# pqpeqr/RL-2048-with-Reinforce-and-Actor-Critic

Hardware: NVIDIA B200
Metric: 2048 env-steps/sec (random-legal batched env stepping, 1M packed boards per GPU) (higher is better)
Workload: dtype u64

## Files before the change

### profiles/sass_pipes.py

```python
#!/usr/bin/env python
import collections, os, re, subprocess, sys

ROOT = os.path.dirname(os.path.dirname(os.path.abspath(__file__)))
DEFAULT_LIB = os.path.join(ROOT, "rl-2048-with-reinforce-and-actor-critic_b200", "libb2048.so")
DEFAULT_KERNELS = ["_ZN2b216step_fast_kernelILi3ELb1ELb1EEEvNS_8StepArgsE"]

ALU = {"LOP3", "LOP", "SHF", "SHL", "SHR", "SEL", "FSEL", "ISETP", "FSETP", "IADD3", "IADD", "VIADD", "VIADDMNMX", "LEA",
       "PRMT", "POPC", "FLO", "BREV", "IMNMX", "VIMNMX", "IABS", "BMSK", "SGXT", "PLOP3", "P2R", "R2P", "MOV", "ICMP",
       "ISCADD", "CS2R"}
FMA = {"IMAD", "FFMA", "FMUL", "FADD", "HFMA2", "HADD2", "HMUL2", "IDP", "IMUL"}
FP64 = {"DADD", "DMUL", "DFMA", "DSETP", "F2F", "F2I", "I2F", "I2FP", "F2FP"}
MEM = {"LDS", "LDG", "STG", "STS", "LD", "ST", "ATOM", "ATOMS", "RED", "REDG", "LDC", "LDL", "STL"}
PIPES = ["alu", "fma", "fp64/conv", "mem", "ctrl", "uniform", "other"]

LINE = re.compile(r"\s*/\*([0-9a-f]{4,})\*/\s+(@!?U?P[T0-9]+\s+)?([A-Z0-9_]+)((?:\.[A-Z0-9_]+)*)\s*([^;]*);")


def pipe(op):
    if op in ALU:
        return "alu"
    if op in FMA:
        return "fma"
    if op in FP64:
        return "fp64/conv"
    if op in MEM:
        return "mem"
    if op in {"BRA", "BSSY", "BSYNC", "EXIT", "NOP", "WARPSYNC", "YIELD", "BAR", "PREEXIT", "CALL", "RET", "BPT"}:
        return "ctrl"
    if op.startswith("U") or op in {"S2UR", "R2UR", "S2R", "CS2R"}:
        return "uniform"
    return "other"


def sass_of(path, kernel):
    out = subprocess.run(["cuobjdump", "-sass", "-fun", kernel, path], capture_output=True, text=True)
    if out.returncode != 0 or "Function" not in out.stdout:
        sys.exit(f"cuobjdump found no function {kernel} in {path}:\n{out.stderr}")
    ins = []
    for line in out.stdout.splitlines():
        m = LINE.match(line)
        if m:
            ins.append((int(m.group(1), 16), m.group(3), m.group(3) + m.group(4), m.group(5), bool(m.group(2))))
    return ins


def regions(ins):
    idx = {a[0]: k for k, a in enumerate(ins)}
    best = None
    for a, op, full, arg, pred in ins:
        if op == "BRA" and pred:
            m = re.search(r"0x([0-9a-f]+)", arg)
            tgt = int(m.group(1), 16) if m else None
            if tgt is not None and tgt < a and tgt in idx and (best is None or a - tgt > best[1] - best[0]):
                best = (tgt, a)
    if best is None:
        sys.exit("no loop found")
    lo, hi = idx[best[0]], idx[best[1]]
    first_st = next((k for k in range(lo, hi + 1) if ins[k][1] in ("STG", "ST")), hi + 1)
    blocks = []
    for k in range(lo, first_st):
        a, op, full, arg, pred = ins[k]
        if op == "BSSY":
            m = re.search(r"(B\d+),\s*0x([0-9a-f]+)", arg)
            end = int(m.group(2), 16)
            if end in idx and idx[end] <= first_st:
                blocks.append((k, idx[end]))
    reset = max(blocks, key=lambda b: b[1] - b[0], default=None)
    in_reset = set(range(reset[0], reset[1] + 1)) if reset else set()
    return {"main": [ins[k] for k in range(lo, first_st) if k not in in_reset],
            "reset": [ins[k] for k in sorted(in_reset)],
            "tail": [ins[k] for k in range(first_st, hi + 1)]}


def main():
    args = [a for a in sys.argv[1:] if a != "-v"]
    verbose = "-v" in sys.argv[1:]
    path = args[0] if args else DEFAULT_LIB
    kernels = args[1:] or DEFAULT_KERNELS
    for kern in kernels:
        regs = regions(sass_of(path, kern))
        print(f"{kern}")
        print(f"{'region':8s} {'instrs':>6s} " + " ".join(f"{p:>9s}" for p in PIPES))
        tot = collections.Counter()
        for name, body in regs.items():
            c = collections.Counter(pipe(x[1]) for x in body)
            tot.update(c)
            print(f"{name:8s} {len(body):6d} " + " ".join(f"{c[p]:9d}" for p in PIPES))
        print(f"{'loop':8s} {sum(tot.values()):6d} " + " ".join(f"{tot[p]:9d}" for p in PIPES))
        if verbose:
            for name, body in regs.items():
                c = collections.Counter(x[2] for x in body)
                print(f"  {name}: " + ", ".join(f"{k} {v}" for k, v in c.most_common()))


if __name__ == "__main__":
    main()
```

### rl-2048-with-reinforce-and-actor-critic_b200/csrc/b2048_env.cu

```cuda
#include <cuda_runtime.h>

#include <cstdio>
#include <cstdlib>

#include "b2048_internal.h"
#include "b2048_ptx.cuh"
#include "b2048_step_fast.cuh"

namespace b2 {

__global__ void build_lut_kernel(uint16_t* __restrict__ lut_left, uint8_t* __restrict__ lut_merge) {
    uint32_t row = blockIdx.x * blockDim.x + threadIdx.x;
    if (row >= 65536u) return;
    uint32_t out, merge;
    row_move_left(row, out, merge);
    lut_left[row] = (uint16_t)out;
    lut_merge[row] = (uint8_t)merge;
}

__global__ void build_small_tables_kernel(uint8_t* __restrict__ small) {
    static_assert(B2048_SMALL_BYTES == B2048_TABLES_BYTES - B2048_LUT_BYTES, "small table size mismatch");
    const uint32_t tid = threadIdx.x;
    if (tid < 256u) small_table_entry_agg(tid, reinterpret_cast<AggEntry*>(small + B2048_SMALL_AGG_OFF)[tid]);
    if (tid < 4u) small_table_entry_sel(tid, reinterpret_cast<SelEntry*>(small + B2048_SMALL_SEL_OFF)[tid]);
    if (tid < 64u) small[B2048_SMALL_ACT_OFF + tid] = (uint8_t)small_table_entry_act(tid >> 2, tid & 3u);
}

__global__ void __launch_bounds__(256) reset_kernel(uint64_t* __restrict__ board, uint32_t* __restrict__ score,
                                                     uint32_t* __restrict__ step, uint8_t* __restrict__ max_exp,
                                                     uint8_t* __restrict__ flags,
                                                     const uint8_t* __restrict__ spawn_replay, int64_t n, uint64_t seed,
                                                     uint64_t gid0, uint32_t t) {
    int64_t stride = (int64_t)gridDim.x * blockDim.x;
    for (int64_t i = (int64_t)blockIdx.x * blockDim.x + threadIdx.x; i < n; i += stride) {
        Board b;
        if (spawn_replay) {
            uint32_t r0 = spawn_replay[2 * i], r1 = spawn_replay[2 * i + 1];
            b = place_kth_empty(Board{0u, 0u}, r0 & 0xFu, (r0 & 0x10u) ? 2u : 1u);
            b = place_kth_empty(b, r1 & 0xFu, (r1 & 0x10u) ? 2u : 1u);
        } else {
            b = reset_board(seed, gid0 + (uint64_t)i, t);
        }
        board[i] = to_u64(b);
        if (score) score[i] = 0u;
        if (step) step[i] = 0u;
        if (max_exp) max_exp[i] = 2u;
        if (flags) flags[i] = (uint8_t)legal_mask(b);
    }
}

__global__ void __launch_bounds__(256) np_seed_kernel(const uint64_t* __restrict__ seeds, b2048_np_rng* __restrict__ rng,
                                                       int64_t n) {
    for (int64_t i = (int64_t)blockIdx.x * blockDim.x + threadIdx.x; i < n; i += (int64_t)gridDim.x * blockDim.x)
        rng[i] = np::seed(seeds[i]);
}

__global__ void __launch_bounds__(256) reset_np_kernel(uint64_t* __restrict__ board, uint32_t* __restrict__ score,
                                                        uint32_t* __restrict__ step, uint8_t* __restrict__ max_exp,
                                                        uint8_t* __restrict__ flags, b2048_np_rng* __restrict__ env_rng,
                                                        int64_t n) {
    for (int64_t i = (int64_t)blockIdx.x * blockDim.x + threadIdx.x; i < n; i += (int64_t)gridDim.x * blockDim.x) {
        b2048_np_rng r = env_rng[i];
        const Board b = np::reset_board(r);
        env_rng[i] = r;
        board[i] = to_u64(b);
        if (score) score[i] = 0u;
        if (step) step[i] = 0u;
        if (max_exp) max_exp[i] = 2u;
        if (flags) flags[i] = (uint8_t)legal_mask(b);
    }
}

struct StepArgs {
    const uint64_t* board_in;
    uint64_t* board_out;
    uint32_t* score;
    uint32_t* step;
    uint8_t* max_exp;
    const uint8_t* action;
    uint8_t* action_out;
    const uint8_t* flags_in;
    const uint8_t* spawn_replay;
    int32_t* ep_len;
    uint32_t ep_t;
    int32_t* merge_sum;
    float* reward;
    double* reward64;
    uint8_t* flags;
    float* obs;
    const uint8_t* tables;
    int64_t n;
    uint64_t seed, gid0;
    uint32_t t;
    b2048_env_cfg cfg;
    PhiloxKeys keys;
    long long* debug_clock;
};

template <bool kSmall, class Args>
__device__ __forceinline__ void stage_tables(uint8_t* smem, const Args& args, uint64_t* mbar) {
    const uint32_t bar = s_u32(mbar);
    if (threadIdx.x == 0) {
        mbar_init(bar, 1);
        mbar_init_fence();
    }
    __syncthreads();
    if (threadIdx.x == 0) {
        mbar_expect_tx(bar, kSmall ? (uint32_t)B2048_TABLES_BYTES : (uint32_t)B2048_LUT_BYTES);
        if (kSmall) bulk_load(s_u32(smem + B2048_LUT_BYTES), args.tables + B2048_LUT_BYTES, (uint32_t)B2048_SMALL_BYTES, bar);
        bulk_load_chunked<32768u>(s_u32(smem), args.tables, (uint32_t)B2048_LUT_BYTES, bar);
    }
}

__device__ __forceinline__ void store_obs16(float* __restrict__ obs, Board nb, int64_t warp_base, int64_t n, int lane,
                                            int obs_mode, float scale) {
#pragma unroll
    for (int s = 0; s < 4; ++s) {
        int src = 8 * s + (lane >> 2);
        uint32_t lo = __shfl_sync(0xFFFFFFFFu, nb.lo, src);
        uint32_t hi = __shfl_sync(0xFFFFFFFFu, nb.hi, src);
        int row = lane & 3;
        uint32_t w = (row & 2) ? hi : lo;
        uint32_t r16 = (w >> (16 * (row & 1))) & 0xFFFFu;
        float v[4];
        encode_row(r16, obs_mode, scale, v);
        int64_t bi = warp_base + src;
        if (bi < n) {
            float4 q = make_float4(v[0], v[1], v[2], v[3]);
            *reinterpret_cast<float4*>(obs + bi * 16 + row * 4) = q;
        }
    }
}

__device__ __forceinline__ void store_obs_onehot(float* __restrict__ obs, Board nb, int64_t warp_base, int64_t n,
                                                 int lane) {
    for (int j = 0; j < 32; ++j) {
        int64_t bi = warp_base + j;
        if (bi >= n) break;
        uint32_t lo = __shfl_sync(0xFFFFFFFFu, nb.lo, j);
        uint32_t hi = __shfl_sync(0xFFFFFFFFu, nb.hi, j);
        uint64_t b = (uint64_t)lo | ((uint64_t)hi << 32);
        float4* dst = reinterpret_cast<float4*>(obs + bi * 272);
#pragma unroll
        for (int q0 = 0; q0 < 96; q0 += 32) {
            int q = q0 + lane;
            if (q < 68) {
                float v[4];
#pragma unroll
                for (int u = 0; u < 4; ++u) {
                    int f = 4 * q + u;
                    int cell = f / 17, ch = f - 17 * cell;
                    int e = (int)((b >> (4 * cell)) & 0xFull);
                    v[u] = (e == ch) ? 1.0f : 0.0f;
                }
                dst[q] = make_float4(v[0], v[1], v[2], v[3]);
            }
        }
    }
}

template <bool kSmemLut, int kThreads, bool kNp>
__device__ __forceinline__ void step_loop(const StepArgs& args, b2048_np_rng* env_rng) {
    extern __shared__ __align__(128) uint8_t smem[];
    __shared__ uint64_t mbar;

    const int tid = threadIdx.x;
    __builtin_assume(tid < kThreads);
    const int lane = tid & 31;
    const uint16_t* lut_left;
    const uint8_t* lut_merge;

    if (kSmemLut) {
        stage_tables<false>(smem, args, &mbar);
        lut_left = reinterpret_cast<const uint16_t*>(smem);
        lut_merge = smem + B2048_LUT_LEFT_BYTES;
    } else {
        lut_left = reinterpret_cast<const uint16_t*>(args.tables);
        lut_merge = args.tables + B2048_LUT_LEFT_BYTES;
    }

    const b2048_env_cfg& cfg = args.cfg;
    StepOpts opt;
    opt.track_step = args.step != nullptr;
    opt.track_max = args.max_exp != nullptr;
    opt.want_sum = cfg.reward_mode == B2048_REWARD_SUM || args.score != nullptr || args.merge_sum != nullptr;

    bool lut_ready = !kSmemLut;
    const int64_t stride = (int64_t)gridDim.x * kThreads;
    for (int64_t base = (int64_t)blockIdx.x * kThreads; base < args.n; base += stride) {
        const int64_t i = base + tid;
        const bool valid = i < args.n;
        StepIO io;
        io.board = Board{0u, 0u};
        io.score = 0u;
        io.step = 0u;
        io.max_exp = 2u;
        io.action = 0u;
        io.mask_in = 0u;
        io.have_mask_in = args.flags_in != nullptr;
        io.replay = 0u;
        if (valid) {
            if (args.spawn_replay) io.replay = args.spawn_replay[i];
            io.board = make_board(args.board_in[i]);
            if (args.score) io.score = args.score[i];
            if (args.step) io.step = args.step[i];
            if (args.max_exp) io.max_exp = args.max_exp[i];
            if (cfg.action_mode == B2048_ACT_BUFFER) io.action = args.action[i];
            if (args.flags_in) io.mask_in = args.flags_in[i];
        }
        if (!lut_ready) {
            mbar_wait(s_u32(&mbar), 0);
            lut_ready = true;
        }
        bool frozen = false;
        Board board_before = io.board;
        if (args.ep_len && valid) frozen = args.ep_len[i] != 0;
        b2048_np_rng rng;
        if constexpr (kNp) {
            if (valid && !frozen) rng = env_rng[i];
        }
        step_one<decltype(lut_left), decltype(lut_merge), kNp>(io, cfg, opt, args.seed, args.gid0 + (uint64_t)i, args.t,
                                                              lut_left, lut_merge, &rng, valid && !frozen);
        if (valid && frozen) {
            uint32_t m = legal_mask(board_before);
            uint32_t f = args.flags_in ? (uint32_t)args.flags_in[i]
                                       : (m | ((m == 0u && (board_before.lo | board_before.hi) != 0u) ? B2048_F_DONE : 0u));
            args.board_out[i] = to_u64(board_before);
            if (args.action_out) args.action_out[i] = 0;
            if (args.merge_sum) args.merge_sum[i] = 0;
            if (args.reward) args.reward[i] = 0.0f;
            if (args.reward64) args.reward64[i] = 0.0;
            args.flags[i] = (uint8_t)(f & ~B2048_F_CHANGED);
            io.board = board_before;
        } else if (valid) {
            if (args.ep_len && (io.flags & (B2048_F_DONE | B2048_F_TRUNC))) args.ep_len[i] = (int32_t)args.ep_t;
            args.board_out[i] = to_u64(io.board);
            if (args.score) args.score[i] = io.score;
            if (args.step) args.step[i] = io.step;
            if (args.max_exp) args.max_exp[i] = (uint8_t)io.max_exp;
            if (args.action_out) args.action_out[i] = (uint8_t)io.action_played;
            if (args.merge_sum) args.merge_sum[i] = io.merge_sum;
            if (args.reward) args.reward[i] = (float)io.reward;
            if (args.reward64) args.reward64[i] = io.reward;
            args.flags[i] = (uint8_t)io.flags;
            if constexpr (kNp) {
                if (io.flags & B2048_F_CHANGED) env_rng[i] = rng;
            }
        }
        if (args.obs != nullptr && cfg.obs_mode != B2048_OBS_NONE) {
            const int64_t warp_base = base + (tid & ~31);
            if (cfg.obs_mode == B2048_OBS_ONEHOT) store_obs_onehot(args.obs, io.board, warp_base, args.n, lane);
            else store_obs16(args.obs, io.board, warp_base, args.n, lane, cfg.obs_mode, cfg.obs_log2_scale);
        }
    }
}

template <bool kSmemLut, int kThreads>
__global__ void __launch_bounds__(kThreads, kSmemLut ? 1 : 2) step_kernel(const __grid_constant__ StepArgs args) {
    step_loop<kSmemLut, kThreads, false>(args, nullptr);
}

template <bool kSmemLut, int kThreads>
__global__ void __launch_bounds__(kThreads, kSmemLut ? 1 : 2) step_np_kernel(const __grid_constant__ StepArgs args,
                                                                              b2048_np_rng* __restrict__ env_rng) {
    step_loop<kSmemLut, kThreads, true>(args, env_rng);
}

template <int kAct, bool kTrack, bool kPlain>
__global__ void __launch_bounds__(1024, 1) step_fast_kernel(const __grid_constant__ StepArgs args) {
    extern __shared__ __align__(128) uint8_t smem[];
    __shared__ uint64_t mbar;
    const int tid = threadIdx.x;
    const bool dbg = args.debug_clock != nullptr && tid == 0 && (blockIdx.x == 0 || blockIdx.x == 147);
    long long* dc = dbg ? args.debug_clock + (blockIdx.x == 0 ? 0 : 16) : nullptr;
    int dci = 0;
    if (dbg) { dc[dci++] = (long long)globaltimer(); dc[dci++] = clock64(); }
    pdl_launch_dependents();
    stage_tables<true>(smem, args, &mbar);
    FastTables T;
    T.left = reinterpret_cast<const uint16_t*>(smem);
    T.merge = smem + B2048_LUT_LEFT_BYTES;
    T.agg = reinterpret_cast<const AggEntry*>(smem + B2048_LUT_BYTES + B2048_SMALL_AGG_OFF);
    T.sel = reinterpret_cast<const SelEntry*>(smem + B2048_LUT_BYTES + B2048_SMALL_SEL_OFF);
    T.act = smem + B2048_LUT_BYTES + B2048_SMALL_ACT_OFF;
    pdl_wait();

    const b2048_env_cfg& cfg = args.cfg;
    if constexpr (kPlain) {
        const uint32_t n = (uint32_t)args.n, stride = gridDim.x * 1024u;
        uint32_t i = blockIdx.x * 1024u + (uint32_t)tid;
        uint2 bw_next = make_uint2(0u, 0u);
        uint32_t act_next = 0u, fin_next = 0u, score_next = 0u, step_next = 0u, max_next = 2u;
        auto request = [&](uint32_t k) {
            bw_next = *reinterpret_cast<const uint2*>(args.board_in + k);
            if (kAct == B2048_ACT_BUFFER) act_next = args.action[k];
            else if (kAct != B2048_ACT_RANDOM_ANY) fin_next = args.flags_in[k];
            if (kTrack) { score_next = args.score[k]; step_next = args.step[k]; max_next = args.max_exp[k]; }
        };
        if (i < n) request(i);
        Rand4 rnd = stream_keyed(args.keys, args.gid0 + (uint64_t)i, args.t, B2048_DOM_STEP);
        mbar_wait(s_u32(&mbar), 0);
        for (; i < n; i += stride) {
            FastIO io;
            io.lo = bw_next.x; io.hi = bw_next.y;
            io.score = score_next; io.step = step_next; io.max_exp = max_next;
            io.action = act_next; io.mask_in = fin_next;
            const uint32_t inext = i + stride;
            if (inext < n) request(inext);
            step_fast_rnd<kAct, kTrack, false>(io, cfg, rnd, args.keys, args.gid0 + (uint64_t)i, args.t, T);
            *reinterpret_cast<uint2*>(args.board_out + i) = make_uint2(io.lo, io.hi);
            if (kTrack) { args.score[i] = io.score; args.step[i] = io.step; args.max_exp[i] = (uint8_t)io.max_exp; }
            args.reward[i] = io.reward;
            args.flags[i] = (uint8_t)io.flags;
            if (inext < n) rnd = stream_keyed(args.keys, args.gid0 + (uint64_t)inext, args.t, B2048_DOM_STEP);
        }
        return;
    }
    bool ready = false;
    const int64_t stride = (int64_t)gridDim.x * 1024;
    int64_t i = (int64_t)blockIdx.x * 1024 + tid;
    uint2 bw_next = make_uint2(0u, 0u);
    uint32_t act_next = 0u, fin_next = 0u;
    if (i < args.n) {
        bw_next = *reinterpret_cast<const uint2*>(args.board_in + i);
        if (kAct == B2048_ACT_BUFFER) act_next = args.action[i];
        if (args.flags_in) fin_next = args.flags_in[i];
    }
    for (; i < args.n; i += stride) {
        FastIO io;
        const uint2 bw = bw_next;
        const uint32_t fin = fin_next;
        io.lo = bw.x; io.hi = bw.y;
        io.score = 0u; io.step = 0u; io.max_exp = 2u; io.mask_in = 0u;
        io.action = act_next;
        const int64_t inext = i + stride;
        if (inext < args.n) {
            bw_next = *reinterpret_cast<const uint2*>(args.board_in + inext);
            if (kAct == B2048_ACT_BUFFER) act_next = args.action[inext];
            if (args.flags_in) fin_next = args.flags_in[inext];
        }
        if (kTrack) { io.score = args.score[i]; io.step = args.step[i]; io.max_exp = args.max_exp[i]; }
        if (kAct == B2048_ACT_RANDOM_LEGAL || kAct == B2048_ACT_PRIORITY)
            io.mask_in = args.flags_in ? fin : legal_mask(Board{io.lo, io.hi});
        bool frozen = false;
        if (args.ep_len) frozen = args.ep_len[i] != 0;
        if (!ready) {
            mbar_wait(s_u32(&mbar), 0);
            ready = true;
            if (dbg) dc[dci++] = clock64();
        }
        if (frozen) {
            uint32_t m = legal_mask(Board{io.lo, io.hi});
            uint32_t f = args.flags_in ? fin : (m | ((m == 0u && (io.lo | io.hi) != 0u) ? B2048_F_DONE : 0u));
            *reinterpret_cast<uint2*>(args.board_out + i) = bw;
            if (args.action_out) args.action_out[i] = 0;
            if (args.merge_sum) args.merge_sum[i] = 0;
            args.reward[i] = 0.0f;
            args.flags[i] = (uint8_t)(f & ~B2048_F_CHANGED);
            continue;
        }
        step_fast<kAct, kTrack>(io, cfg, args.keys, args.seed, args.gid0 + (uint64_t)i, args.t, T);
        if (args.ep_len && (io.flags & (B2048_F_DONE | B2048_F_TRUNC))) args.ep_len[i] = (int32_t)args.ep_t;
        *reinterpret_cast<uint2*>(args.board_out + i) = make_uint2(io.lo, io.hi);
        if (kTrack) { args.score[i] = io.score; args.step[i] = io.step; args.max_exp[i] = (uint8_t)io.max_exp; }
        if (args.action_out) args.action_out[i] = (uint8_t)io.action;
        if (args.merge_sum) args.merge_sum[i] = io.merge_sum;
        args.reward[i] = io.reward;
        args.flags[i] = (uint8_t)io.flags;
        if (dbg && dci < 12) dc[dci++] = clock64();
    }
    if (dbg) { const unsigned long long gt = globaltimer(); dc[14] = clock64(); dc[15] = (long long)gt; }
}

template <int kAct, bool kTrack, bool kPlain>
static cudaError_t launch_fast_one(int grid, size_t smem, cudaStream_t s, const StepArgs& a, bool pdl) {
    cudaLaunchConfig_t lc = {};
    lc.gridDim = dim3((unsigned)grid); lc.blockDim = dim3(1024); lc.dynamicSmemBytes = smem; lc.stream = s;
    cudaLaunchAttribute at[1];
    at[0].id = cudaLaunchAttributeProgrammaticStreamSerialization;
    at[0].val.programmaticStreamSerializationAllowed = 1;
    lc.attrs = at; lc.numAttrs = pdl ? 1u : 0u;
    return cudaLaunchKernelEx(&lc, step_fast_kernel<kAct, kTrack, kPlain>, a);
}
template <int kAct>
static cudaError_t launch_fast(bool track, int grid, size_t smem, cudaStream_t s, const StepArgs& a, bool pdl) {
    const bool plain = a.ep_len == nullptr && a.action_out == nullptr && a.merge_sum == nullptr && a.debug_clock == nullptr &&
                       (kAct == B2048_ACT_BUFFER || kAct == B2048_ACT_RANDOM_ANY || a.flags_in != nullptr) &&
                       a.n < ((int64_t)1 << 31) - (int64_t)grid * 1024 &&
                       !cfg_is_shaped(a.cfg);
    if (plain) return track ? launch_fast_one<kAct, true, true>(grid, smem, s, a, pdl) : launch_fast_one<kAct, false, true>(grid, smem, s, a, pdl);
    return track ? launch_fast_one<kAct, true, false>(grid, smem, s, a, pdl) : launch_fast_one<kAct, false, false>(grid, smem, s, a, pdl);
}

struct StepNArgs {
    uint64_t* board;
    uint32_t* score;
    uint32_t* step;
    uint8_t* max_exp;
    uint8_t* flags;
    float* reward_last;
    float* reward_sum;
    int32_t* episodes;
    const uint8_t* tables;
    int64_t n;
    int32_t n_steps, flags_valid;
    uint64_t seed, gid0;
    uint32_t t;
    b2048_env_cfg cfg;
    PhiloxKeys keys;
};

template <int kAct, bool kTrack, bool kShaped>
__global__ void __launch_bounds__(1024, 1) step_fast_n_kernel(const __grid_constant__ StepNArgs args) {
    extern __shared__ __align__(128) uint8_t smem[];
    __shared__ uint64_t mbar;
    const int tid = threadIdx.x;
    stage_tables<true>(smem, args, &mbar);
    FastTables T;
    T.left = reinterpret_cast<const uint16_t*>(smem);
    T.merge = smem + B2048_LUT_LEFT_BYTES;
    T.agg = reinterpret_cast<const AggEntry*>(smem + B2048_LUT_BYTES + B2048_SMALL_AGG_OFF);
    T.sel = reinterpret_cast<const SelEntry*>(smem + B2048_LUT_BYTES + B2048_SMALL_SEL_OFF);
    T.act = smem + B2048_LUT_BYTES + B2048_SMALL_ACT_OFF;
    const b2048_env_cfg& cfg = args.cfg;
    bool ready = false;
    const int64_t stride = (int64_t)gridDim.x * 1024;
    for (int64_t i = (int64_t)blockIdx.x * 1024 + tid; i < args.n; i += stride) {
        FastIO io;
        const uint2 bw = *reinterpret_cast<const uint2*>(args.board + i);
        io.lo = bw.x; io.hi = bw.y;
        io.score = 0u; io.step = 0u; io.max_exp = 2u; io.action = 0u;
        if (kTrack) { io.score = args.score[i]; io.step = args.step[i]; io.max_exp = args.max_exp[i]; }
        io.mask_in = args.flags_valid ? (uint32_t)args.flags[i] : legal_mask(Board{io.lo, io.hi});
        io.flags = io.mask_in;
        io.reward = 0.0f;
        if (!ready) {
            mbar_wait(s_u32(&mbar), 0);
            ready = true;
        }
        float rsum = 0.0f;
        int32_t eps = 0;
        const uint64_t gid = args.gid0 + (uint64_t)i;
        for (int32_t k = 0; k < args.n_steps; ++k) {
            io.mask_in = io.flags & 0xFu;
            step_fast<kAct, kTrack, kShaped>(io, cfg, args.keys, args.seed, gid, args.t + (uint32_t)k, T);
            rsum += io.reward;
            eps += (io.flags & (B2048_F_DONE | B2048_F_TRUNC)) ? 1 : 0;
        }
        *reinterpret_cast<uint2*>(args.board + i) = make_uint2(io.lo, io.hi);
        if (kTrack) { args.score[i] = io.score; args.step[i] = io.step; args.max_exp[i] = (uint8_t)io.max_exp; }
        args.flags[i] = (uint8_t)io.flags;
        if (args.reward_last) args.reward_last[i] = io.reward;
        if (args.reward_sum) args.reward_sum[i] += rsum;
        if (args.episodes) args.episodes[i] += eps;
    }
}

__global__ void __launch_bounds__(256) move_kernel(const uint64_t* __restrict__ board_in, uint64_t* __restrict__ board_out,
                                                    const uint8_t* __restrict__ action, int32_t* __restrict__ merge_sum,
                                                    uint8_t* __restrict__ merge_info, uint8_t* __restrict__ flags,
                                                    const uint8_t* __restrict__ tables, int64_t n) {
    const uint16_t* lut_left = reinterpret_cast<const uint16_t*>(tables);
    const uint8_t* lut_merge = tables + B2048_LUT_LEFT_BYTES;
    int64_t stride = (int64_t)gridDim.x * blockDim.x;
    for (int64_t i = (int64_t)blockIdx.x * blockDim.x + threadIdx.x; i < n; i += stride) {
        Board b = make_board(board_in[i]);
        MoveResult mv = move_board(b, action[i] & 3u, lut_left, lut_merge);
        MergeStats ms = merge_stats(mv.merge, true, false);
        uint32_t mask = legal_mask(mv.board);
        bool changed = (mv.board.lo != b.lo) | (mv.board.hi != b.hi);
        bool done = (mask == 0u) & ((mv.board.lo | mv.board.hi) != 0u);
        board_out[i] = to_u64(mv.board);
        if (merge_sum) merge_sum[i] = (int32_t)ms.sum;
        if (merge_info) *reinterpret_cast<uint32_t*>(merge_info + 4 * i) = mv.merge;
        if (flags)
            flags[i] = (uint8_t)(mask | (changed ? B2048_F_CHANGED : 0u) | (done ? B2048_F_DONE : 0u) |
                                 (ms.overflow ? B2048_F_OVERFLOW : 0u));
    }
}

__global__ void __launch_bounds__(256) obs_kernel(const uint64_t* __restrict__ board, float* __restrict__ obs, int obs_mode,
                                                   float scale, int64_t n) {
    const int lane = threadIdx.x & 31;
    int64_t stride = (int64_t)gridDim.x * blockDim.x;
    for (int64_t base = (int64_t)blockIdx.x * blockDim.x; base < n; base += stride) {
        int64_t i = base + threadIdx.x;
        Board b = i < n ? make_board(board[i]) : Board{0u, 0u};
        int64_t warp_base = base + (threadIdx.x & ~31);
        if (obs_mode == B2048_OBS_ONEHOT) store_obs_onehot(obs, b, warp_base, n, lane);
        else store_obs16(obs, b, warp_base, n, lane, obs_mode, scale);
    }
}

struct SymVariant {
    uint64_t perm;
    uint32_t amap;
    uint32_t mperm;
};
__constant__ SymVariant kSym[8] = {
    {0xFEDCBA9876543210ull, 0xE4u, 0xE4u}, {0xC840D951EA62FB73ull, 0x93u, 0x39u},
    {0x0123456789ABCDEFull, 0x4Eu, 0x4Eu}, {0x37BF26AE159D048Cull, 0x39u, 0x93u},
    {0xCDEF89AB45670123ull, 0x6Cu, 0x6Cu}, {0xFB73EA62D951C840ull, 0x1Bu, 0x1Bu},
    {0x32107654BA98FEDCull, 0xC6u, 0xC6u}, {0x048C159D26AE37BFull, 0xB1u, 0xB1u},
};

__global__ void __launch_bounds__(256) symmetries_kernel(const uint64_t* __restrict__ board, const uint8_t* __restrict__ flags,
                                                          const uint8_t* __restrict__ action, uint64_t* __restrict__ board_out,
                                                          uint8_t* __restrict__ flags_out, uint8_t* __restrict__ action_out,
                                                          int64_t rows, int64_t n) {
    const int64_t total = rows * n;
    for (int64_t e = (int64_t)blockIdx.x * blockDim.x + threadIdx.x; e < total; e += (int64_t)gridDim.x * blockDim.x) {
        const int64_t r = e / n, i = e - r * n;
        const uint64_t b = board ? board[e] : 0ull;
        const uint32_t f = flags ? flags[e] : 0u, a = action ? (action[e] & 3u) : 0u;
#pragma unroll
        for (int v = 0; v < 8; ++v) {
            const SymVariant sv = kSym[v];
            const int64_t o = r * 8 * n + (int64_t)v * n + i;
            if (board_out) {
                uint64_t nb = 0;
#pragma unroll
                for (int c = 0; c < 16; ++c) nb |= ((b >> (4 * (uint32_t)((sv.perm >> (4 * c)) & 0xFull))) & 0xFull) << (4 * c);
                board_out[o] = nb;
            }
            if (flags_out) {
                uint32_t nf = f & 0xF0u;
#pragma unroll
                for (int k = 0; k < 4; ++k) nf |= ((f >> ((sv.mperm >> (2 * k)) & 3u)) & 1u) << k;
                flags_out[o] = (uint8_t)nf;
            }
            if (action_out) action_out[o] = (uint8_t)((sv.amap >> (2 * a)) & 3u);
        }
    }
}

static int grid_for(int64_t n, int threads, int num_sms, int per_sm) {
    int64_t blocks = (n + threads - 1) / threads;
    int64_t cap = (int64_t)num_sms * per_sm;
    if (blocks > cap) blocks = cap;
    if (blocks < 1) blocks = 1;
    return (int)blocks;
}

}

using namespace b2;

extern "C" int b2048_create(b2048_handle** out) {
    B2_REQUIRE(out != nullptr, "b2048_create: out is NULL");
    b2048_handle* h = new b2048_handle();
    B2_CUDA(cudaGetDevice(&h->device));
    B2_CUDA(cudaDeviceGetAttribute(&h->num_sms, cudaDevAttrMultiProcessorCount, h->device));
    B2_CUDA(cudaDeviceGetAttribute(&h->smem_optin, cudaDevAttrMaxSharedMemoryPerBlockOptin, h->device));
    B2_CUDA(cudaMalloc(&h->d_tables, B2048_TABLES_BYTES));
    build_lut_kernel<<<256, 256>>>(reinterpret_cast<uint16_t*>(h->d_tables), h->d_tables + B2048_LUT_LEFT_BYTES);
    build_small_tables_kernel<<<1, 256>>>(h->d_tables + B2048_LUT_BYTES);
    B2_CUDA(cudaGetLastError());
    B2_CUDA(cudaDeviceSynchronize());
    if (h->smem_optin >= B2048_LUT_BYTES) {
        B2_CUDA(cudaFuncSetAttribute(step_kernel<true, 1024>, cudaFuncAttributeMaxDynamicSharedMemorySize,
                                     B2048_LUT_BYTES));
        B2_CUDA(cudaFuncSetAttribute(step_np_kernel<true, 1024>, cudaFuncAttributeMaxDynamicSharedMemorySize,
                                     B2048_LUT_BYTES));
    }
    if (h->smem_optin >= B2048_TABLES_BYTES) {
#define B2_SET(A, TR)                                                                                                       \
    B2_CUDA(cudaFuncSetAttribute(step_fast_kernel<A, TR, false>, cudaFuncAttributeMaxDynamicSharedMemorySize, B2048_TABLES_BYTES)); \
    B2_CUDA(cudaFuncSetAttribute(step_fast_kernel<A, TR, true>, cudaFuncAttributeMaxDynamicSharedMemorySize, B2048_TABLES_BYTES))
        B2_SET(B2048_ACT_BUFFER, true); B2_SET(B2048_ACT_BUFFER, false);
        B2_SET(B2048_ACT_RANDOM_LEGAL, true); B2_SET(B2048_ACT_RANDOM_LEGAL, false);
        B2_SET(B2048_ACT_RANDOM_ANY, true); B2_SET(B2048_ACT_RANDOM_ANY, false);
        B2_SET(B2048_ACT_PRIORITY, true); B2_SET(B2048_ACT_PRIORITY, false);
#define B2_SET_N(A, TR)                                                                                                               \
    do {                                                                                                                              \
        B2_CUDA(cudaFuncSetAttribute(step_fast_n_kernel<A, TR, false>, cudaFuncAttributeMaxDynamicSharedMemorySize, B2048_TABLES_BYTES)); \
        B2_CUDA(cudaFuncSetAttribute(step_fast_n_kernel<A, TR, true>, cudaFuncAttributeMaxDynamicSharedMemorySize, B2048_TABLES_BYTES));  \
    } while (0)
        B2_SET_N(B2048_ACT_RANDOM_LEGAL, true); B2_SET_N(B2048_ACT_RANDOM_LEGAL, false);
        B2_SET_N(B2048_ACT_RANDOM_ANY, true); B2_SET_N(B2048_ACT_RANDOM_ANY, false);
        B2_SET_N(B2048_ACT_PRIORITY, true); B2_SET_N(B2048_ACT_PRIORITY, false);
#undef B2_SET_N
#undef B2_SET
    }
    *out = h;
    return B2048_OK;
}

extern "C" int b2048_destroy(b2048_handle* h) {
    if (!h) return B2048_OK;
    cudaFree(h->d_tables);
    if (h->tc_image) cudaFree(h->tc_image);
    if (h->hp_image) cudaFree(h->hp_image);
    if (h->gen_image) cudaFree(h->gen_image);
    if (h->dbg_clock) cudaFree(h->dbg_clock);
    if (h->dbg_progress) cudaFreeHost(h->dbg_progress);
    delete h;
    return B2048_OK;
}

extern "C" int b2048_get_row_lut(b2048_handle* h, uint16_t* lut_left_host, uint8_t* lut_merge_host) {
    B2_REQUIRE(h != nullptr, "b2048_get_row_lut: handle is NULL");
    if (lut_left_host) B2_CUDA(cudaMemcpy(lut_left_host, h->d_tables, B2048_LUT_LEFT_BYTES, cudaMemcpyDeviceToHost));
    if (lut_merge_host)
        B2_CUDA(cudaMemcpy(lut_merge_host, h->d_tables + B2048_LUT_LEFT_BYTES, B2048_LUT_MERGE_BYTES,
                           cudaMemcpyDeviceToHost));
    return B2048_OK;
}

extern "C" int b2048_reset_many(b2048_handle* h, uint64_t* board, uint32_t* score, uint32_t* step, uint8_t* max_exp,
                                uint8_t* flags, const uint8_t* spawn_replay, int64_t n, uint64_t seed, uint64_t gid0,
                                uint32_t t, void* stream) {
    B2_REQUIRE(h != nullptr, "b2048_reset_many: handle is NULL");
    B2_REQUIRE(n >= 0, "b2048_reset_many: n < 0");
    B2_REQUIRE(board != nullptr || n == 0, "b2048_reset_many: board is NULL");
    if (n == 0) return B2048_OK;
    reset_kernel<<<grid_for(n, 256, h->num_sms, 8), 256, 0, (cudaStream_t)stream>>>(board, score, step, max_exp, flags,
                                                                                   spawn_replay, n, seed, gid0, t);
    B2_CUDA(cudaGetLastError());
    return B2048_OK;
}

extern "C" int b2048_np_rng_seed(const uint64_t* seeds, b2048_np_rng* rng, int64_t n, void* stream) {
    B2_REQUIRE(n >= 0, "b2048_np_rng_seed: n < 0");
    if (n == 0) return B2048_OK;
    B2_REQUIRE(seeds && rng, "b2048_np_rng_seed: seeds / rng is NULL");
    const int64_t blocks = (n + 255) / 256;
    np_seed_kernel<<<(unsigned)(blocks < 65536 ? blocks : 65536), 256, 0, (cudaStream_t)stream>>>(seeds, rng, n);
    B2_CUDA(cudaGetLastError());
    return B2048_OK;
}

extern "C" int b2048_reset_many_np(b2048_handle* h, uint64_t* board, uint32_t* score, uint32_t* step, uint8_t* max_exp,
                                   uint8_t* flags, b2048_np_rng* env_rng, int64_t n, void* stream) {
    B2_REQUIRE(h != nullptr, "b2048_reset_many_np: handle is NULL");
    B2_REQUIRE(n >= 0, "b2048_reset_many_np: n < 0");
    if (n == 0) return B2048_OK;
    B2_REQUIRE(board && env_rng, "b2048_reset_many_np: board / env_rng is NULL");
    reset_np_kernel<<<grid_for(n, 256, h->num_sms, 8), 256, 0, (cudaStream_t)stream>>>(board, score, step, max_exp, flags,
                                                                                       env_rng, n);
    B2_CUDA(cudaGetLastError());
    return B2048_OK;
}

int b2::launch_step_np(b2048_handle* h, const uint64_t* board_in, uint64_t* board_out, uint32_t* score, uint32_t* step,
                   uint8_t* max_exp, const uint8_t* action, const uint8_t* flags_in, const b2048_env_cfg* cfg, float* reward,
                   uint8_t* flags, int32_t* ep_len, uint32_t ep_t, int64_t n, b2048_np_rng* env_rng, cudaStream_t s) {
    StepArgs a = {};
    a.board_in = board_in; a.board_out = board_out; a.score = score; a.step = step; a.max_exp = max_exp;
    a.action = action; a.flags_in = flags_in; a.ep_len = ep_len; a.ep_t = ep_t;
    a.reward = reward; a.flags = flags; a.tables = h->d_tables; a.n = n; a.cfg = *cfg;
    if (h->smem_optin >= B2048_LUT_BYTES && n >= (int64_t)32768) {
        step_np_kernel<true, 1024><<<grid_for(n, 1024, h->num_sms, 1), 1024, B2048_LUT_BYTES, s>>>(a, env_rng);
    } else {
        step_np_kernel<false, 256><<<grid_for(n, 256, h->num_sms, 8), 256, 0, s>>>(a, env_rng);
    }
    B2_CUDA(cudaGetLastError());
    return B2048_OK;
}

extern "C" int b2048_step_many(b2048_handle* h, const uint64_t* board_in, uint64_t* board_out, uint32_t* score,
                               uint32_t* step, uint8_t* max_exp, const uint8_t* action, uint8_t* action_out,
                               const uint8_t* flags_in, const uint8_t* spawn_replay, const b2048_env_cfg* cfg,
                               int32_t* merge_sum, float* reward,
                               double* reward64, uint8_t* flags, float* obs, int32_t* ep_len, uint32_t ep_t, int64_t n,
                               uint64_t seed, uint64_t gid0, uint32_t t, void* stream) {
    B2_REQUIRE(h != nullptr, "b2048_step_many: handle is NULL");
    B2_REQUIRE(cfg != nullptr, "b2048_step_many: cfg is NULL");
    B2_REQUIRE(n >= 0, "b2048_step_many: n < 0");
    if (n == 0) return B2048_OK;
    B2_REQUIRE(board_in && board_out && flags, "b2048_step_many: board_in/board_out/flags must not be NULL");
    B2_REQUIRE(cfg->reward_mode == B2048_REWARD_SUM || cfg->reward_mode == B2048_REWARD_LOG2,
               "b2048_step_many: unsupported reward mode");
    B2_REQUIRE(cfg->bonus_mode >= B2048_BONUS_OFF && cfg->bonus_mode <= B2048_BONUS_LOG2,
               "b2048_step_many: unsupported bonus mode");
    B2_REQUIRE(cfg->obs_mode >= B2048_OBS_NONE && cfg->obs_mode <= B2048_OBS_ONEHOT,
               "b2048_step_many: unsupported obs_mode");
    B2_REQUIRE(cfg->action_mode >= B2048_ACT_BUFFER && cfg->action_mode <= B2048_ACT_PRIORITY,
               "b2048_step_many: unsupported action_mode");
    B2_REQUIRE(cfg->action_mode != B2048_ACT_BUFFER || action != nullptr,
               "b2048_step_many: action buffer required for B2048_ACT_BUFFER");
    StepArgs a;
    a.board_in = board_in; a.board_out = board_out; a.score = score; a.step = step; a.max_exp = max_exp;
    a.action = action; a.action_out = action_out; a.flags_in = flags_in; a.spawn_replay = spawn_replay; a.ep_len = ep_len; a.ep_t = ep_t;
    a.merge_sum = merge_sum;
    a.reward = reward; a.reward64 = reward64; a.flags = flags; a.obs = obs; a.tables = h->d_tables;
    a.n = n; a.seed = seed; a.gid0 = gid0; a.t = t; a.cfg = *cfg; a.keys = make_keys(seed);
    cudaStream_t s = (cudaStream_t)stream;
    a.debug_clock = debug_clock_begin(h, B2048_DBG_STEP_CLOCKS, s);
    const bool use_smem = h->smem_optin >= B2048_LUT_BYTES && n >= (int64_t)32768;
    const bool all_track = score && step && max_exp, none_track = !score && !step && !max_exp;
    const bool fast = h->smem_optin >= B2048_TABLES_BYTES && n >= (int64_t)32768 && (all_track || none_track) &&
                      cfg->use_action_mask && (cfg->bonus_mode == B2048_BONUS_OFF || all_track) && reward != nullptr &&
                      reward64 == nullptr && spawn_replay == nullptr && (obs == nullptr || cfg->obs_mode == B2048_OBS_NONE) &&
                      !(h->debug & (1u << B2048_DBG_NO_FAST_STEP));
    if (fast) {
        int grid = grid_for(n, 1024, h->num_sms, 1);
        const bool pdl = !(h->debug & (1u << B2048_DBG_NO_PDL));
        cudaError_t e;
        if (cfg->action_mode == B2048_ACT_BUFFER) e = launch_fast<B2048_ACT_BUFFER>(all_track, grid, B2048_TABLES_BYTES, s, a, pdl);
        else if (cfg->action_mode == B2048_ACT_RANDOM_LEGAL) e = launch_fast<B2048_ACT_RANDOM_LEGAL>(all_track, grid, B2048_TABLES_BYTES, s, a, pdl);
        else if (cfg->action_mode == B2048_ACT_PRIORITY) e = launch_fast<B2048_ACT_PRIORITY>(all_track, grid, B2048_TABLES_BYTES, s, a, pdl);
        else e = launch_fast<B2048_ACT_RANDOM_ANY>(all_track, grid, B2048_TABLES_BYTES, s, a, pdl);
        B2_CUDA(e);
    } else if (use_smem) {
        int grid = grid_for(n, 1024, h->num_sms, 1);
        step_kernel<true, 1024><<<grid, 1024, B2048_LUT_BYTES, s>>>(a);
    } else {
        int grid = grid_for(n, 256, h->num_sms, 8);
        step_kernel<false, 256><<<grid, 256, 0, s>>>(a);
    }
    B2_CUDA(cudaGetLastError());
    if (a.debug_clock && fast) {
        long long hb[32];
        { int st = debug_clock_read(h, hb, 32, s); if (st != B2048_OK) return st; }
        for (int c = 0; c < 2; ++c) {
            long long* d = hb + 16 * c;
            fprintf(stderr, "[step clock] cta %d: start@%lld ns, staged +%lld cyc, iters:", c ? 147 : 0, d[0] - hb[0], d[2] - d[1]);
            for (int k = 3; k < 12 && d[k]; ++k) fprintf(stderr, " %lld", d[k] - d[k - 1]);
            fprintf(stderr, " | total %lld cyc, %lld ns\n", d[14] - d[1], d[15] - d[0]);
        }
    }
    return B2048_OK;
}

extern "C" int b2048_symmetries(b2048_handle* h, const uint64_t* board, const uint8_t* flags, const uint8_t* action,
                                uint64_t* board_out, uint8_t* flags_out, uint8_t* action_out, int64_t rows, int64_t n,
                                void* stream) {
    B2_REQUIRE(h != nullptr, "b2048_symmetries: handle is NULL");
    B2_REQUIRE(rows >= 0 && n >= 0, "b2048_symmetries: negative size");
    if (rows == 0 || n == 0) return B2048_OK;
    B2_REQUIRE((board == nullptr) == (board_out == nullptr) && (flags == nullptr) == (flags_out == nullptr) &&
                   (action == nullptr) == (action_out == nullptr),
               "b2048_symmetries: every input needs its output buffer and vice versa");
    symmetries_kernel<<<grid_for(rows * n, 256, h->num_sms, 8), 256, 0, (cudaStream_t)stream>>>(
        board, flags, action, board_out, flags_out, action_out, rows, n);
    B2_CUDA(cudaGetLastError());
    return B2048_OK;
}

extern "C" int b2048_step_many_n(b2048_handle* h, uint64_t* board, uint32_t* score, uint32_t* step, uint8_t* max_exp,
                                 uint8_t* flags, int32_t flags_valid, const b2048_env_cfg* cfg, float* reward_last,
                                 float* reward_sum, int32_t* episodes, int64_t n, int32_t n_steps, uint64_t seed,
                                 uint64_t gid0, uint32_t t, void* stream) {
    B2_REQUIRE(h != nullptr && cfg != nullptr, "b2048_step_many_n: handle / cfg is NULL");
    B2_REQUIRE(n >= 0 && n_steps >= 0, "b2048_step_many_n: negative size");
    if (n == 0 || n_steps == 0) return B2048_OK;
    B2_REQUIRE(board && flags, "b2048_step_many_n: board / flags must not be NULL");
    B2_REQUIRE(cfg->action_mode == B2048_ACT_RANDOM_LEGAL || cfg->action_mode == B2048_ACT_RANDOM_ANY ||
                   cfg->action_mode == B2048_ACT_PRIORITY,
               "b2048_step_many_n: needs a device-side action mode (random_legal, random_any or priority)");
    const bool all_track = score && step && max_exp, none_track = !score && !step && !max_exp;
    const bool ok = h->smem_optin >= B2048_TABLES_BYTES && (all_track || none_track) && cfg->use_action_mask &&
                    (cfg->bonus_mode == B2048_BONUS_OFF || all_track) &&
                    (cfg->reward_mode == B2048_REWARD_SUM || cfg->reward_mode == B2048_REWARD_LOG2);
    if (!ok)
        return fail(B2048_ERR_UNSUPPORTED,
                    "b2048_step_many_n: implemented for action-mask-on configurations (the new-max-tile bonus needs the "
                    "tracked counters) with score / step / max_exp all present or all absent; call "
                    "b2048_step_many n_steps times otherwise");
    StepNArgs a;
    a.board = board; a.score = score; a.step = step; a.max_exp = max_exp; a.flags = flags; a.reward_last = reward_last;
    a.reward_sum = reward_sum; a.episodes = episodes; a.tables = h->d_tables; a.n = n; a.n_steps = n_steps;
    a.flags_valid = flags_valid; a.seed = seed; a.gid0 = gid0; a.t = t; a.cfg = *cfg; a.keys = make_keys(seed);
    const int grid = grid_for(n, 1024, h->num_sms, 1);
    cudaStream_t s = (cudaStream_t)stream;
    const bool shaped = cfg_is_shaped(*cfg);
#define B2_LAUNCH_N(A)                                                                                      \
    do {                                                                                                    \
        if (all_track && shaped) step_fast_n_kernel<A, true, true><<<grid, 1024, B2048_TABLES_BYTES, s>>>(a);    \
        else if (all_track) step_fast_n_kernel<A, true, false><<<grid, 1024, B2048_TABLES_BYTES, s>>>(a);        \
        else if (shaped) step_fast_n_kernel<A, false, true><<<grid, 1024, B2048_TABLES_BYTES, s>>>(a);           \
        else step_fast_n_kernel<A, false, false><<<grid, 1024, B2048_TABLES_BYTES, s>>>(a);                      \
    } while (0)
    if (cfg->action_mode == B2048_ACT_RANDOM_LEGAL) B2_LAUNCH_N(B2048_ACT_RANDOM_LEGAL);
    else if (cfg->action_mode == B2048_ACT_PRIORITY) B2_LAUNCH_N(B2048_ACT_PRIORITY);
    else B2_LAUNCH_N(B2048_ACT_RANDOM_ANY);
#undef B2_LAUNCH_N
    B2_CUDA(cudaGetLastError());
    return B2048_OK;
}

extern "C" int b2048_move_many(b2048_handle* h, const uint64_t* board_in, uint64_t* board_out, const uint8_t* action,
                               int32_t* merge_sum, uint8_t* merge_info, uint8_t* flags, int64_t n, void* stream) {
    B2_REQUIRE(h != nullptr, "b2048_move_many: handle is NULL");
    B2_REQUIRE(n >= 0, "b2048_move_many: n < 0");
    if (n == 0) return B2048_OK;
    B2_REQUIRE(board_in && board_out && action, "b2048_move_many: board_in/board_out/action must not be NULL");
    move_kernel<<<grid_for(n, 256, h->num_sms, 8), 256, 0, (cudaStream_t)stream>>>(board_in, board_out, action, merge_sum,
                                                                                  merge_info, flags, h->d_tables, n);
    B2_CUDA(cudaGetLastError());
    return B2048_OK;
}

extern "C" int b2048_encode_obs(const uint64_t* board, float* obs, int32_t obs_mode, float obs_log2_scale, int64_t n,
                                void* stream) {
    B2_REQUIRE(n >= 0, "b2048_encode_obs: n < 0");
    B2_REQUIRE(obs_mode >= B2048_OBS_RAW && obs_mode <= B2048_OBS_ONEHOT, "b2048_encode_obs: unsupported obs_mode");
    if (n == 0) return B2048_OK;
    B2_REQUIRE(board && obs, "b2048_encode_obs: board/obs must not be NULL");
    int dev = 0, sms = 148;
    B2_CUDA(cudaGetDevice(&dev));
    B2_CUDA(cudaDeviceGetAttribute(&sms, cudaDevAttrMultiProcessorCount, dev));
    obs_kernel<<<grid_for(n, 256, sms, 8), 256, 0, (cudaStream_t)stream>>>(board, obs, obs_mode, obs_log2_scale, n);
    B2_CUDA(cudaGetLastError());
    return B2048_OK;
}
```

Baseline: 59.53 billion.

## Process two boards per thread in plain fast step path with vectorized IO

Replaces the plain specialization of the fast step kernel with a new pair kernel that runs 512 threads per block, each stepping two adjacent boards per iteration. Loads and stores use wider vector accesses (uint4 boards, uint2 score/step, 16-bit packed flags/actions) and two independent step chains per thread to raise ILP. The launch path adds alignment checks and handles an odd trailing board separately. The cost is fewer resident threads per SM and higher register pressure, and it adds slope-timing and SASS-counting scripts.

```diff
diff --git a/profiles/run_step_slope.py b/profiles/run_step_slope.py
--- /dev/null
+++ b/profiles/run_step_slope.py
@@ -0,0 +1,70 @@
+#!/usr/bin/env python
+import argparse
+import json
+import os
+import subprocess
+import sys
+
+ROOT = os.path.dirname(os.path.dirname(os.path.abspath(__file__)))
+sys.path.insert(0, ROOT)
+
+
+def gpu_info():
+    try:
+        q = subprocess.run(["nvidia-smi", "--query-gpu=name,power.limit,clocks.max.sm", "--format=csv,noheader"],
+                           capture_output=True, text=True, timeout=30)
+        return q.stdout.strip().splitlines()[0] if q.returncode == 0 and q.stdout.strip() else None
+    except (OSError, subprocess.SubprocessError):
+        return None
+
+
+def time_launch(b2048, torch, n, K, R):
+    from bench import RUNNER_ENV
+    envs = [b2048.Batched2048Env(n, b2048.Game2048EnvConfig(**RUNNER_ENV), seed=0xB200 + r, gid0=0) for r in range(R)]
+    for e in envs:
+        e.reset_many()
+        e.step_many_n(64, action_mode="random_legal", auto_reset=True)
+    for k in range(max(10, R)):
+        envs[k % R].step_many(action_mode="random_legal", auto_reset=True)
+    t0, t1 = torch.cuda.Event(enable_timing=True), torch.cuda.Event(enable_timing=True)
+    torch.cuda.synchronize()
+    torch.cuda._sleep(2_000_000)
+    t0.record()
+    for k in range(K):
+        envs[k % R].step_many(action_mode="random_legal", auto_reset=True)
+    t1.record()
+    torch.cuda.synchronize()
+    return t0.elapsed_time(t1) * 1e3 / K
+
+
+def main():
+    ap = argparse.ArgumentParser()
+    ap.add_argument("--steps", type=int, default=2000)
+    ap.add_argument("--batches", type=int, default=12)
+    ap.add_argument("--kmax", type=int, default=7)
+    ap.add_argument("--out")
+    args = ap.parse_args()
+    import numpy as np
+    import torch
+    import b2048
+    if not torch.cuda.is_available():
+        sys.exit("run_step_slope.py needs a CUDA device")
+    per_iter = torch.cuda.get_device_properties(0).multi_processor_count * 1024
+    ks = list(range(1, args.kmax + 1))
+    us = [time_launch(b2048, torch, k * per_iter, args.steps, args.batches) for k in ks]
+    b, a = np.polyfit(ks, us, 1)
+    resid = np.asarray(us) - (a + b * np.asarray(ks))
+    line = {"gpu": gpu_info(), "boards_per_iteration": per_iter, "steps": args.steps, "batches": args.batches,
+            "us_per_launch": {str(k * per_iter): round(u, 3) for k, u in zip(ks, us)},
+            "fit_us": {"a_fixed": round(float(a), 3), "b_per_iteration": round(float(b), 3),
+                       "max_abs_residual": round(float(np.abs(resid).max()), 3)},
+            "ns_per_board_step_marginal": round(float(b) * 1e3 / per_iter, 5)}
+    print(json.dumps(line))
+    if args.out:
+        os.makedirs(os.path.dirname(os.path.abspath(args.out)), exist_ok=True)
+        with open(args.out, "w") as f:
+            f.write(json.dumps(line) + "\n")
+
+
+if __name__ == "__main__":
+    main()
diff --git a/profiles/sass_pipes.py b/profiles/sass_pipes.py
--- a/profiles/sass_pipes.py
+++ b/profiles/sass_pipes.py
@@ -3,7 +3,8 @@
 
 ROOT = os.path.dirname(os.path.dirname(os.path.abspath(__file__)))
 DEFAULT_LIB = os.path.join(ROOT, "rl-2048-with-reinforce-and-actor-critic_b200", "libb2048.so")
-DEFAULT_KERNELS = ["_ZN2b216step_fast_kernelILi3ELb1ELb1EEEvNS_8StepArgsE"]
+DEFAULT_KERNELS = ["_ZN2b216step_pair_kernelILi1ELb1EEEvNS_8StepArgsE"]
+RESET_WARP_FRAC = 0.25
 
 ALU = {"LOP3", "LOP", "SHF", "SHL", "SHR", "SEL", "FSEL", "ISETP", "FSETP", "IADD3", "IADD", "VIADD", "VIADDMNMX", "LEA",
        "PRMT", "POPC", "FLO", "BREV", "IMNMX", "VIMNMX", "IABS", "BMSK", "SGXT", "PLOP3", "P2R", "R2P", "MOV", "ICMP",
@@ -57,19 +58,22 @@
         sys.exit("no loop found")
     lo, hi = idx[best[0]], idx[best[1]]
     first_st = next((k for k in range(lo, hi + 1) if ins[k][1] in ("STG", "ST")), hi + 1)
-    blocks = []
-    for k in range(lo, first_st):
+    resets, k = [], lo
+    while k < first_st:
         a, op, full, arg, pred = ins[k]
         if op == "BSSY":
             m = re.search(r"(B\d+),\s*0x([0-9a-f]+)", arg)
             end = int(m.group(2), 16)
             if end in idx and idx[end] <= first_st:
-                blocks.append((k, idx[end]))
-    reset = max(blocks, key=lambda b: b[1] - b[0], default=None)
-    in_reset = set(range(reset[0], reset[1] + 1)) if reset else set()
+                if any("c[0x3]" in ins[q][3] for q in range(k, idx[end])):
+                    resets.append((k, idx[end]))
+                k = idx[end]
+                continue
+        k += 1
+    in_reset = {q for b0, b1 in resets for q in range(b0, b1)}
     return {"main": [ins[k] for k in range(lo, first_st) if k not in in_reset],
             "reset": [ins[k] for k in sorted(in_reset)],
-            "tail": [ins[k] for k in range(first_st, hi + 1)]}
+            "tail": [ins[k] for k in range(first_st, hi + 1)]}, max(1, len(resets))
 
 
 def main():
@@ -78,15 +82,19 @@
     path = args[0] if args else DEFAULT_LIB
     kernels = args[1:] or DEFAULT_KERNELS
     for kern in kernels:
-        regs = regions(sass_of(path, kern))
-        print(f"{kern}")
-        print(f"{'region':8s} {'instrs':>6s} " + " ".join(f"{p:>9s}" for p in PIPES))
-        tot = collections.Counter()
-        for name, body in regs.items():
-            c = collections.Counter(pipe(x[1]) for x in body)
-            tot.update(c)
-            print(f"{name:8s} {len(body):6d} " + " ".join(f"{c[p]:9d}" for p in PIPES))
-        print(f"{'loop':8s} {sum(tot.values()):6d} " + " ".join(f"{tot[p]:9d}" for p in PIPES))
+        regs, boards = regions(sass_of(path, kern))
+        print(f"{kern}: {boards} board(s) per iteration")
+        print(f"{'region':16s} {'instrs':>7s} " + " ".join(f"{p:>9s}" for p in PIPES))
+        counts = {name: collections.Counter(pipe(x[1]) for x in body) for name, body in regs.items()}
+        tot = sum(counts.values(), collections.Counter())
+        row = lambda name, c: print(f"{name:16s} {sum(c[p] for p in PIPES):7.1f} " + " ".join(f"{c[p]:9.1f}" for p in PIPES))
+        for name, c in counts.items():
+            row(name, c)
+        row("loop", tot)
+        per = {name: {p: c[p] / boards for p in PIPES} for name, c in counts.items()}
+        for name in counts:
+            row(name + " / board", per[name])
+        row("avg board-step", {p: per["main"][p] + per["tail"][p] + RESET_WARP_FRAC * per["reset"][p] for p in PIPES})
         if verbose:
             for name, body in regs.items():
                 c = collections.Counter(x[2] for x in body)
diff --git a/rl-2048-with-reinforce-and-actor-critic_b200/csrc/b2048_env.cu b/rl-2048-with-reinforce-and-actor-critic_b200/csrc/b2048_env.cu
--- a/rl-2048-with-reinforce-and-actor-critic_b200/csrc/b2048_env.cu
+++ b/rl-2048-with-reinforce-and-actor-critic_b200/csrc/b2048_env.cu
@@ -266,7 +266,7 @@
     step_loop<kSmemLut, kThreads, true>(args, env_rng);
 }
 
-template <int kAct, bool kTrack, bool kPlain>
+template <int kAct, bool kTrack>
 __global__ void __launch_bounds__(1024, 1) step_fast_kernel(const __grid_constant__ StepArgs args) {
     extern __shared__ __align__(128) uint8_t smem[];
     __shared__ uint64_t mbar;
@@ -286,36 +286,6 @@
     pdl_wait();
 
     const b2048_env_cfg& cfg = args.cfg;
-    if constexpr (kPlain) {
-        const uint32_t n = (uint32_t)args.n, stride = gridDim.x * 1024u;
-        uint32_t i = blockIdx.x * 1024u + (uint32_t)tid;
-        uint2 bw_next = make_uint2(0u, 0u);
-        uint32_t act_next = 0u, fin_next = 0u, score_next = 0u, step_next = 0u, max_next = 2u;
-        auto request = [&](uint32_t k) {
-            bw_next = *reinterpret_cast<const uint2*>(args.board_in + k);
-            if (kAct == B2048_ACT_BUFFER) act_next = args.action[k];
-            else if (kAct != B2048_ACT_RANDOM_ANY) fin_next = args.flags_in[k];
-            if (kTrack) { score_next = args.score[k]; step_next = args.step[k]; max_next = args.max_exp[k]; }
-        };
-        if (i < n) request(i);
-        Rand4 rnd = stream_keyed(args.keys, args.gid0 + (uint64_t)i, args.t, B2048_DOM_STEP);
-        mbar_wait(s_u32(&mbar), 0);
-        for (; i < n; i += stride) {
-            FastIO io;
-            io.lo = bw_next.x; io.hi = bw_next.y;
-            io.score = score_next; io.step = step_next; io.max_exp = max_next;
-            io.action = act_next; io.mask_in = fin_next;
-            const uint32_t inext = i + stride;
-            if (inext < n) request(inext);
-            step_fast_rnd<kAct, kTrack, false>(io, cfg, rnd, args.keys, args.gid0 + (uint64_t)i, args.t, T);
-            *reinterpret_cast<uint2*>(args.board_out + i) = make_uint2(io.lo, io.hi);
-            if (kTrack) { args.score[i] = io.score; args.step[i] = io.step; args.max_exp[i] = (uint8_t)io.max_exp; }
-            args.reward[i] = io.reward;
-            args.flags[i] = (uint8_t)io.flags;
-            if (inext < n) rnd = stream_keyed(args.keys, args.gid0 + (uint64_t)inext, args.t, B2048_DOM_STEP);
-        }
-        return;
-    }
     bool ready = false;
     const int64_t stride = (int64_t)gridDim.x * 1024;
     int64_t i = (int64_t)blockIdx.x * 1024 + tid;
@@ -372,24 +342,119 @@
     if (dbg) { const unsigned long long gt = globaltimer(); dc[14] = clock64(); dc[15] = (long long)gt; }
 }
 
-template <int kAct, bool kTrack, bool kPlain>
-static cudaError_t launch_fast_one(int grid, size_t smem, cudaStream_t s, const StepArgs& a, bool pdl) {
+template <int kAct, bool kTrack>
+__global__ void __launch_bounds__(512, 1) step_pair_kernel(const __grid_constant__ StepArgs args) {
+    extern __shared__ __align__(128) uint8_t smem[];
+    __shared__ uint64_t mbar;
+    pdl_launch_dependents();
+    stage_tables<true>(smem, args, &mbar);
+    FastTables T;
+    T.left = reinterpret_cast<const uint16_t*>(smem);
+    T.merge = smem + B2048_LUT_LEFT_BYTES;
+    T.agg = reinterpret_cast<const AggEntry*>(smem + B2048_LUT_BYTES + B2048_SMALL_AGG_OFF);
+    T.sel = reinterpret_cast<const SelEntry*>(smem + B2048_LUT_BYTES + B2048_SMALL_SEL_OFF);
+    T.act = smem + B2048_LUT_BYTES + B2048_SMALL_ACT_OFF;
+    pdl_wait();
+
+    const b2048_env_cfg& cfg = args.cfg;
+    const PhiloxKeys& keys = args.keys;
+    const uint64_t gid0 = args.gid0;
+    const uint32_t t = args.t;
+    const uint32_t n = (uint32_t)args.n, npairs = n >> 1, stride = gridDim.x * 512u;
+    uint32_t j = blockIdx.x * 512u + threadIdx.x;
+    const uint4* bin = reinterpret_cast<const uint4*>(args.board_in) + j;
+    const uint16_t* in8 = reinterpret_cast<const uint16_t*>(kAct == B2048_ACT_BUFFER ? args.action : args.flags_in) + j;
+    uint2* score = reinterpret_cast<uint2*>(args.score) + j;
+    uint2* step = reinterpret_cast<uint2*>(args.step) + j;
+    uint16_t* max_exp = reinterpret_cast<uint16_t*>(args.max_exp) + j;
+    uint4* bout = reinterpret_cast<uint4*>(args.board_out) + j;
+    float2* reward = reinterpret_cast<float2*>(args.reward) + j;
+    uint16_t* flags = reinterpret_cast<uint16_t*>(args.flags) + j;
+    uint4 bw_next = make_uint4(0u, 0u, 0u, 0u);
+    uint2 score_next = make_uint2(0u, 0u), step_next = make_uint2(0u, 0u);
+    uint32_t in8_next = 0u, max_next = 0x0202u;
+    if (j < npairs) {
+        bw_next = *bin;
+        if (kAct != B2048_ACT_RANDOM_ANY) in8_next = *in8;
+        if (kTrack) { score_next = *score; step_next = *step; max_next = *max_exp; }
+    }
+    Rand4 rnd0 = stream_keyed(keys, gid0 + 2u * j, t, B2048_DOM_STEP);
+    Rand4 rnd1 = stream_keyed(keys, gid0 + 2u * j + 1u, t, B2048_DOM_STEP);
+    mbar_wait(s_u32(&mbar), 0);
+    for (; j < npairs; j += stride) {
+        FastIO a, b;
+        a.lo = bw_next.x; a.hi = bw_next.y; b.lo = bw_next.z; b.hi = bw_next.w;
+        a.score = score_next.x; b.score = score_next.y; a.step = step_next.x; b.step = step_next.y;
+        a.max_exp = max_next & 0xFFu; b.max_exp = max_next >> 8;
+        a.action = a.mask_in = in8_next; b.action = b.mask_in = in8_next >> 8;
+        const uint32_t jn = j + stride;
+        bin += stride; in8 += stride;
+        uint2* const score_n = score + stride;
+        uint2* const step_n = step + stride;
+        uint16_t* const max_exp_n = max_exp + stride;
+        if (jn < npairs) {
+            bw_next = *bin;
+            if (kAct != B2048_ACT_RANDOM_ANY) in8_next = *in8;
+            if (kTrack) { score_next = *score_n; step_next = *step_n; max_next = *max_exp_n; }
+        }
+        const uint64_t gid = gid0 + 2u * j;
+        step_fast_rnd<kAct, kTrack, false>(a, cfg, rnd0, keys, gid, t, T);
+        step_fast_rnd<kAct, kTrack, false>(b, cfg, rnd1, keys, gid + 1u, t, T);
+        *bout = make_uint4(a.lo, a.hi, b.lo, b.hi);
+        if (kTrack) {
+            *score = make_uint2(a.score, b.score);
+            *step = make_uint2(a.step, b.step);
+            *max_exp = (uint16_t)(a.max_exp | (b.max_exp << 8));
+        }
+        *reward = make_float2(a.reward, b.reward);
+        *flags = (uint16_t)(a.flags | (b.flags << 8));
+        bout += stride; reward += stride; flags += stride;
+        score = score_n; step = step_n; max_exp = max_exp_n;
+        if (jn < npairs) {
+            rnd0 = stream_keyed(keys, gid0 + 2u * jn, t, B2048_DOM_STEP);
+            rnd1 = stream_keyed(keys, gid0 + 2u * jn + 1u, t, B2048_DOM_STEP);
+        }
+    }
+    if ((n & 1u) && j == npairs) {
+        const uint32_t i = n - 1u;
+        FastIO io;
+        const uint2 bw = *reinterpret_cast<const uint2*>(args.board_in + i);
+        io.lo = bw.x; io.hi = bw.y;
+        io.score = kTrack ? args.score[i] : 0u;
+        io.step = kTrack ? args.step[i] : 0u;
+        io.max_exp = kTrack ? args.max_exp[i] : 2u;
+        io.action = kAct == B2048_ACT_BUFFER ? args.action[i] : 0u;
+        io.mask_in = kAct != B2048_ACT_BUFFER && kAct != B2048_ACT_RANDOM_ANY ? args.flags_in[i] : 0u;
+        step_fast_rnd<kAct, kTrack, false>(io, cfg, stream_keyed(keys, gid0 + i, t, B2048_DOM_STEP), keys, gid0 + i, t, T);
+        *reinterpret_cast<uint2*>(args.board_out + i) = make_uint2(io.lo, io.hi);
+        if (kTrack) { args.score[i] = io.score; args.step[i] = io.step; args.max_exp[i] = (uint8_t)io.max_exp; }
+        args.reward[i] = io.reward;
+        args.flags[i] = (uint8_t)io.flags;
+    }
+}
+
+static cudaError_t launch_pdl(void (*kernel)(StepArgs), unsigned threads, int grid, size_t smem, cudaStream_t s,
+                              const StepArgs& a, bool pdl) {
     cudaLaunchConfig_t lc = {};
-    lc.gridDim = dim3((unsigned)grid); lc.blockDim = dim3(1024); lc.dynamicSmemBytes = smem; lc.stream = s;
+    lc.gridDim = dim3((unsigned)grid); lc.blockDim = dim3(threads); lc.dynamicSmemBytes = smem; lc.stream = s;
     cudaLaunchAttribute at[1];
     at[0].id = cudaLaunchAttributeProgrammaticStreamSerialization;
     at[0].val.programmaticStreamSerializationAllowed = 1;
     lc.attrs = at; lc.numAttrs = pdl ? 1u : 0u;
-    return cudaLaunchKernelEx(&lc, step_fast_kernel<kAct, kTrack, kPlain>, a);
-}
+    return cudaLaunchKernelEx(&lc, kernel, a);
+}
+static bool aligned(const void* p, uintptr_t bytes) { return ((uintptr_t)p & (bytes - 1u)) == 0u; }
 template <int kAct>
 static cudaError_t launch_fast(bool track, int grid, size_t smem, cudaStream_t s, const StepArgs& a, bool pdl) {
     const bool plain = a.ep_len == nullptr && a.action_out == nullptr && a.merge_sum == nullptr && a.debug_clock == nullptr &&
                        (kAct == B2048_ACT_BUFFER || kAct == B2048_ACT_RANDOM_ANY || a.flags_in != nullptr) &&
                        a.n < ((int64_t)1 << 31) - (int64_t)grid * 1024 &&
-                       !cfg_is_shaped(a.cfg);
-    if (plain) return track ? launch_fast_one<kAct, true, true>(grid, smem, s, a, pdl) : launch_fast_one<kAct, false, true>(grid, smem, s, a, pdl);
-    return track ? launch_fast_one<kAct, true, false>(grid, smem, s, a, pdl) : launch_fast_one<kAct, false, false>(grid, smem, s, a, pdl);
+                       !cfg_is_shaped(a.cfg) &&
+                       aligned(a.board_in, 16) && aligned(a.board_out, 16) && aligned(a.reward, 8) && aligned(a.flags, 2) &&
+                       (kAct == B2048_ACT_RANDOM_ANY || aligned(kAct == B2048_ACT_BUFFER ? a.action : a.flags_in, 2)) &&
+                       (!track || (aligned(a.score, 8) && aligned(a.step, 8) && aligned(a.max_exp, 2)));
+    if (plain) return launch_pdl(track ? step_pair_kernel<kAct, true> : step_pair_kernel<kAct, false>, 512, grid, smem, s, a, pdl);
+    return launch_pdl(track ? step_fast_kernel<kAct, true> : step_fast_kernel<kAct, false>, 1024, grid, smem, s, a, pdl);
 }
 
 struct StepNArgs {
@@ -565,8 +630,8 @@
     }
     if (h->smem_optin >= B2048_TABLES_BYTES) {
 #define B2_SET(A, TR)                                                                                                       \
-    B2_CUDA(cudaFuncSetAttribute(step_fast_kernel<A, TR, false>, cudaFuncAttributeMaxDynamicSharedMemorySize, B2048_TABLES_BYTES)); \
-    B2_CUDA(cudaFuncSetAttribute(step_fast_kernel<A, TR, true>, cudaFuncAttributeMaxDynamicSharedMemorySize, B2048_TABLES_BYTES))
+    B2_CUDA(cudaFuncSetAttribute(step_fast_kernel<A, TR>, cudaFuncAttributeMaxDynamicSharedMemorySize, B2048_TABLES_BYTES)); \
+    B2_CUDA(cudaFuncSetAttribute(step_pair_kernel<A, TR>, cudaFuncAttributeMaxDynamicSharedMemorySize, B2048_TABLES_BYTES))
         B2_SET(B2048_ACT_BUFFER, true); B2_SET(B2048_ACT_BUFFER, false);
         B2_SET(B2048_ACT_RANDOM_LEGAL, true); B2_SET(B2048_ACT_RANDOM_LEGAL, false);
         B2_SET(B2048_ACT_RANDOM_ANY, true); B2_SET(B2048_ACT_RANDOM_ANY, false);
```

Measured after the change: 60.95 billion (median of 6 runs). 1.02x the previous value.
